# levi106/kvedge

Hardware: AMD Instinct MI355X
Metric: images/sec ResNet-50 edge module at 1/2/4/8 MI355X; VM boot-to-ready sec (higher is better)
Workload: dtype bf16; 1 GPU; model=resnet50, global_batch=1280, per_gpu_batch=1280, image_size=224, parallelism=dp1, backend=none, hip_graph=True, streams=2, microbatch=0, mb_blocks=3

## Files before the change

csrc/kernels/conv_seam.hip:

```cpp
#include "common.h"
#include "kvedge_kernels.h"

namespace kvedge {
namespace {

constexpr int kSmOOB = 0x7ffffff0;
constexpr int kSmLdsMax = 160 * 1024;

template <int I>
struct SmIC {
  static constexpr int value = I;
};
template <int N, int I = 0, class F>
__device__ __forceinline__ void sm_static_for(F&& f) {
  if constexpr (I < N) {
    f(SmIC<I>{});
    sm_static_for<N, I + 1>(f);
  }
}

template <int N>
__device__ __forceinline__ void sm_wait_vm() {
  static_assert(N >= 0 && N <= 63, "vmcnt field");
  asm volatile("s_waitcnt vmcnt(%0)" ::"n"(N) : "memory");
}

template <int SY, int SZ, int D, int RD, int KB, int NA>
struct SmSched {
  static constexpr int SPT = SY + SZ;
  static constexpr int kB = KB, kR = 2, kS = 2, kA = NA;
  static constexpr int kFar = 12;
  static constexpr int kTiles = kFar + 2;
  static constexpr int wait(int kind, int idx) {
    long endB[kTiles * SPT + D + 2] = {};
    long endR[kTiles + RD + 2] = {};
    long pos = kA;
    for (int t = 0; t < RD - 1; ++t) endR[t] = (pos += kR);
    for (int s = 0; s < D - 1; ++s) endB[s] = (pos += kB);
    for (int t = 0; t < kTiles; ++t) {
      for (int j = 0; j < SPT; ++j) {
        const int s = t * SPT + j;
        if (j == SY) {
          if (kind == 1 && idx == t) return (int)(pos - endR[t]);
          pos += kS;
        }
        if (kind == 0 && idx == s) return (int)(pos - endB[s]);
        if (kind == 2 && idx == s) return D >= 3 ? (int)(pos - endB[s + 1]) : -1;
        endB[s + D - 1] = (pos += kB);
        if (j == 0) endR[t + RD - 1] = (pos += kR);
      }
    }
    return -1;
  }
  static constexpr int wB(int t, int j) { return wait(0, t * SPT + j); }
  static constexpr int wE(int t) { return wait(1, t); }
  static constexpr int wXB(int t, int j) { return wait(2, t * SPT + j); }
  static constexpr int steady_from() {
    int t0 = 0;
    for (int t = 0; t < kFar; ++t) {
      bool same = wE(t) == wE(kFar);
      for (int j = 0; j < SPT; ++j)
        same = same && wB(t, j) == wB(kFar, j) && wXB(t, j) == wXB(kFar, j);
      if (!same) t0 = t + 1;
    }
    return t0;
  }
  static constexpr int kSteady = steady_from();
  static constexpr int safe_B(int j) {
    int m = wB(kFar, j);
    for (int t = 0; t <= kSteady; ++t) m = wB(t, j) < m ? wB(t, j) : m;
    return m;
  }
  static constexpr int safe_XB(int j) {
    int m = wXB(kFar, j);
    for (int t = 0; t <= kSteady; ++t) m = wXB(t, j) < m ? wXB(t, j) : m;
    return m;
  }
  static constexpr int safe_E() {
    int m = wE(kFar);
    for (int t = 0; t <= kSteady; ++t) m = wE(t) < m ? wE(t) : m;
    return m;
  }
  static constexpr bool ok(bool xp = false) {
    for (int t = 0; t <= kFar; ++t) {
      if (wE(t) < 0 || wE(t) > 63) return false;
      for (int j = 0; j < SPT; ++j) {
        if (wB(t, j) < 0 || wB(t, j) > 63) return false;
        if (xp && (wXB(t, j) < 0 || wXB(t, j) > 63)) return false;
      }
    }
    return kSteady < kFar;
  }
};

__device__ __forceinline__ int sm_sw(int r) { return (r >> 1) & 7; }

__device__ __forceinline__ void sm_lds_barrier() {
  asm volatile("s_waitcnt lgkmcnt(0)" ::: "memory");
  __builtin_amdgcn_s_barrier();
  asm volatile("" ::: "memory");
}

template <int NC3, int NZC, int D, int RD, int NW = 8, int KS2 = 1, bool AREG = false,
          bool XP = false>
__global__ __launch_bounds__(64 * NW, NW == 4 ? 2 : 1) void conv_seam_kernel(const KvConvParams p, int ntiles) {
  static_assert(NW == 4 || NW == 8, "waves");
  static_assert(NC3 % KS2 == 0 && NZC % KS2 == 0, "whole chunks per ring stage");
  constexpr int SY = NC3 / KS2, SZ = NZC / KS2, BPW = 8 / NW;
  using S = SmSched<SY, SZ, D, RD, KS2 * BPW, AREG ? 0 : 2 * NC3>;
  static_assert(S::ok(XP), "counted-wait schedule out of range or not periodic");
  constexpr int SPT = S::SPT, BM = 16 * NW, NT = 64 * NW;
  static_assert(!XP || (AREG && D >= 3 && SPT % 2 == 0),
                "XP: A in VGPRs, stage s + 1 issued before step s, register sets by step parity");
  constexpr int A_BYTES = AREG ? 0 : NC3 * BM * 128, B_CHUNK = 64 * 128, B_STAGE = KS2 * B_CHUNK;
  constexpr int R_SLOT = BM * 64 * 2;
  constexpr int B_OFF = A_BYTES, R_OFF = B_OFF + D * B_STAGE, BIAS_OFF = R_OFF + RD * R_SLOT;
  constexpr int BIAS_ROUND = NW * 1024;
  extern __shared__ __attribute__((aligned(16))) char sm_smem[];
  char* const lds = sm_smem;

  const int tid = threadIdx.x, lane = tid & 63;
  const int wv = __builtin_amdgcn_readfirstlane(tid >> 6);
  const int wm = wv >> 1, wn = wv & 1;
  const int nbm = (p.M + BM - 1) / BM;
  const int m0 = xcd_remap(blockIdx.x, nbm) * BM;
  const int Cout = p.Cout, N1 = p.n_t;
  const int b1_off = BIAS_OFF + ((Cout * 4 + BIAS_ROUND - 1) / BIAS_ROUND) * BIAS_ROUND;

  const kv_i32x4 rx = kv_rsrc4(p.x, p.M * p.ldx * 2);
  const kv_i32x4 rw3 = kv_rsrc4(p.w, Cout * p.Kpad * 2);
  const kv_i32x4 rw1 = kv_rsrc4(p.w_t, N1 * Cout * 2);
  const kv_i32x4 rr = kv_rsrc4(p.res, p.M * p.ldr * 2);
  const kv_i32x4 rb3 = kv_rsrc4(p.bias, Cout * 4);
  const kv_i32x4 rb1 = kv_rsrc4(p.bias_t, N1 * 4);
  const __amdgpu_buffer_rsrc_t ry =
      __builtin_amdgcn_make_buffer_rsrc(p.y, (short)0, p.M * p.ldy * 2, 0x00020000);
  const __amdgpu_buffer_rsrc_t rz =
      __builtin_amdgcn_make_buffer_rsrc(p.z, (short)0, p.M * p.ldz * 2, 0x00020000);

  const int lrow = lane >> 3, pch = lane & 7;
  int arow_off[2], r_src[2], lc8[2];
#pragma unroll
  for (int i = 0; i < 2; ++i) {
    const int row = (wv * 2 + i) * 8 + lrow;
    const int lc = pch ^ sm_sw(row);
    lc8[i] = lc * 8;
    const int m = m0 + row;
    arow_off[i] = m < p.M ? (m * p.ldx + p.x_coff + lc * 8) * 2 : kSmOOB;
    r_src[i] = m < p.M ? (m * p.ldr + p.r_coff + lc * 8) * 2 : kSmOOB;
  }
  int w3_src[BPW], w1_src[BPW], brow[BPW];
#pragma unroll
  for (int i = 0; i < BPW; ++i) {
    brow[i] = (wv * BPW + i) * 8 + lrow;
    const int bch = (pch ^ sm_sw(brow[i])) * 8;
    w3_src[i] = (brow[i] * p.Kpad + bch) * 2;
    w1_src[i] = (brow[i] * Cout + bch) * 2;
  }

  auto issue_B = [&](int tt, auto JJ) __attribute__((always_inline)) {
    constexpr int jj = decltype(JJ)::value;
    const int s = tt * SPT + jj;
    char* dst = lds + B_OFF + (s % D) * B_STAGE;
#pragma unroll
    for (int c = 0; c < KS2; ++c)
#pragma unroll
      for (int i = 0; i < BPW; ++i) {
        char* d = dst + c * B_CHUNK + (wv * BPW + i) * 1024;
        if constexpr (jj < SY) {
          const int n = tt * 64 + brow[i];
          const int v = (tt < ntiles && n < Cout) ? w3_src[i] + (tt * 64 * p.Kpad + (jj * KS2 + c) * 64) * 2 : kSmOOB;
          kv_lds_dma16(rw3, d, v);
        } else {
          const int zc = (jj - SY) * KS2 + c;
          const int zr = zc * 64 + brow[i];
          const int v = (tt < ntiles && zr < N1) ? w1_src[i] + (zc * 64 * Cout + tt * 64) * 2 : kSmOOB;
          kv_lds_dma16(rw1, d, v);
        }
      }
  };
  auto issue_R = [&](int tt) __attribute__((always_inline)) {
    char* dst = lds + R_OFF + (tt % RD) * R_SLOT;
#pragma unroll
    for (int i = 0; i < 2; ++i) {
      const int n = tt * 64 + lc8[i];
      const int v = (tt < ntiles && n < Cout && r_src[i] != kSmOOB) ? r_src[i] + tt * 128 : kSmOOB;
      kv_lds_dma16_nt(rr, dst + (wv * 2 + i) * 1024, v);
    }
  };

  for (int i = 0; i < (Cout * 4 + BIAS_ROUND - 1) / BIAS_ROUND; ++i) {
    const int off = (i * NW + wv) * 1024;
    kv_lds_dma16(rb3, lds + BIAS_OFF + off, off + lane * 16);
  }
  for (int i = 0; i < (N1 * 4 + BIAS_ROUND - 1) / BIAS_ROUND; ++i) {
    const int off = (i * NW + wv) * 1024;
    kv_lds_dma16(rb1, lds + b1_off + off, off + lane * 16);
  }
  typedef unsigned int sm_u32x4 __attribute__((ext_vector_type(4)));
  sm_u32x4 araw[AREG ? NC3 : 1][2][2];
  const int fr = lane & 15, fh = lane >> 4;
  if constexpr (AREG) {
#pragma unroll
    for (int kc = 0; kc < NC3; ++kc)
#pragma unroll
      for (int ks = 0; ks < 2; ++ks)
#pragma unroll
        for (int tm = 0; tm < 2; ++tm) {
          const int m = m0 + wm * 32 + tm * 16 + fr;
          const int k = kc * 64 + ks * 32 + fh * 8;
          const int off = (m < p.M && k < p.Cin) ? (m * p.ldx + p.x_coff + k) * 2 : kSmOOB;
          asm volatile("buffer_load_dwordx4 %0, %1, %2, 0 offen"
                       : "=v"(araw[kc][ks][tm]) : "v"(off), "s"(rx) : "memory");
        }
  }
  if constexpr (!AREG) {
#pragma unroll
    for (int kc = 0; kc < NC3; ++kc)
#pragma unroll
      for (int i = 0; i < 2; ++i) {
        char* dst = lds + kc * (BM * 128) + (wv * 2 + i) * 1024;
        const int v = (arow_off[i] != kSmOOB && kc * 64 + lc8[i] < p.Cin) ? arow_off[i] + kc * 128 : kSmOOB;
        kv_lds_dma16_nt(rx, dst, v);
      }
  }
#pragma unroll
  for (int t = 0; t < RD - 1; ++t) issue_R(t);
  sm_static_for<D - 1>([&](auto JJ) __attribute__((always_inline)) {
    constexpr int s = decltype(JJ)::value;
    issue_B(s / SPT, SmIC<s % SPT>{});
  });
  bf16x8 areg[AREG ? NC3 : 1][2][2];
  if constexpr (AREG) {
    sm_wait_vm<(RD - 1) * S::kR + (D - 1) * S::kB>();
#pragma unroll
    for (int kc = 0; kc < NC3; ++kc)
#pragma unroll
      for (int ks = 0; ks < 2; ++ks)
#pragma unroll
        for (int tm = 0; tm < 2; ++tm) {
          asm volatile("" : "+v"(araw[kc][ks][tm]));
          areg[kc][ks][tm] = __builtin_bit_cast(bf16x8, araw[kc][ks][tm]);
        }
  }

  floatx4 acc[2][2];
  floatx4 accz[NZC][2][2];
#pragma unroll
  for (int zc = 0; zc < NZC; ++zc)
#pragma unroll
    for (int a = 0; a < 2; ++a)
#pragma unroll
      for (int b = 0; b < 2; ++b) accz[zc][a][b] = floatx4{0.f, 0.f, 0.f, 0.f};

  auto mma64 = [&](const char* As, const char* Bs, floatx4 (&c)[2][2]) __attribute__((always_inline)) {
#pragma unroll
    for (int ks = 0; ks < 2; ++ks) {
      const int q = ks * 4 + fh;
      bf16x8 af[2], bfg[2];
#pragma unroll
      for (int tm = 0; tm < 2; ++tm) {
        const int row = wm * 32 + tm * 16 + fr;
        af[tm] = *reinterpret_cast<const bf16x8*>(As + row * 128 + ((q ^ sm_sw(row)) << 4));
      }
#pragma unroll
      for (int tn = 0; tn < 2; ++tn) {
        const int row = wn * 32 + tn * 16 + fr;
        bfg[tn] = *reinterpret_cast<const bf16x8*>(Bs + row * 128 + ((q ^ sm_sw(row)) << 4));
      }
#pragma unroll
      for (int tn = 0; tn < 2; ++tn)
#pragma unroll
        for (int tm = 0; tm < 2; ++tm)
          c[tn][tm] = __builtin_amdgcn_mfma_f32_16x16x32_bf16(bfg[tn], af[tm], c[tn][tm], 0, 0, 0);
    }
  };

  auto mma64r = [&](int kc_unused, const bf16x8 (&a)[2][2], const char* Bs, floatx4 (&c)[2][2])
      __attribute__((always_inline)) {
#pragma unroll
    for (int ks = 0; ks < 2; ++ks) {
      const int q = ks * 4 + fh;
      bf16x8 bfg[2];
#pragma unroll
      for (int tn = 0; tn < 2; ++tn) {
        const int row = wn * 32 + tn * 16 + fr;
        bfg[tn] = *reinterpret_cast<const bf16x8*>(Bs + row * 128 + ((q ^ sm_sw(row)) << 4));
      }
#pragma unroll
      for (int tn = 0; tn < 2; ++tn)
#pragma unroll
        for (int tm = 0; tm < 2; ++tm)
          c[tn][tm] = __builtin_amdgcn_mfma_f32_16x16x32_bf16(bfg[tn], a[ks][tm], c[tn][tm], 0, 0, 0);
    }
  };

  bf16x8 bset[XP ? 2 : 1][XP ? KS2 : 1][2][2];
  auto read_B = [&](bf16x8 (&dst)[XP ? KS2 : 1][2][2], const char* Bs) __attribute__((always_inline)) {
#pragma unroll
    for (int c = 0; c < (XP ? KS2 : 1); ++c)
#pragma unroll
      for (int ks = 0; ks < 2; ++ks)
#pragma unroll
        for (int tn = 0; tn < 2; ++tn) {
          const int row = wn * 32 + tn * 16 + fr, q = ks * 4 + fh;
          dst[c][ks][tn] =
              *reinterpret_cast<const bf16x8*>(Bs + c * B_CHUNK + row * 128 + ((q ^ sm_sw(row)) << 4));
        }
  };
  auto mma_xr = [&](const bf16x8 (&b)[2][2], const bf16x8 (&a)[2][2], floatx4 (&c)[2][2])
      __attribute__((always_inline)) {
#pragma unroll
    for (int ks = 0; ks < 2; ++ks)
#pragma unroll
      for (int tn = 0; tn < 2; ++tn)
#pragma unroll
        for (int tm = 0; tm < 2; ++tm)
          c[tn][tm] = __builtin_amdgcn_mfma_f32_16x16x32_bf16(b[ks][tn], a[ks][tm], c[tn][tm], 0, 0, 0);
  };
  auto mma_xl = [&](const bf16x8 (&b)[2][2], const char* As, floatx4 (&c)[2][2])
      __attribute__((always_inline)) {
#pragma unroll
    for (int ks = 0; ks < 2; ++ks) {
      const int q = ks * 4 + fh;
      bf16x8 af[2];
#pragma unroll
      for (int tm = 0; tm < 2; ++tm) {
        const int row = wm * 32 + tm * 16 + fr;
        af[tm] = *reinterpret_cast<const bf16x8*>(As + row * 128 + ((q ^ sm_sw(row)) << 4));
      }
#pragma unroll
      for (int tn = 0; tn < 2; ++tn)
#pragma unroll
        for (int tm = 0; tm < 2; ++tm)
          c[tn][tm] = __builtin_amdgcn_mfma_f32_16x16x32_bf16(b[ks][tn], af[tm], c[tn][tm], 0, 0, 0);
    }
  };

  dispatch_act(p.act, true, [&](auto A1, auto A2) __attribute__((always_inline)) {
    constexpr int act1 = decltype(A1)::value, act2 = decltype(A2)::value;
    for (int t = 0; t < ntiles; ++t) {
      const bool warm = t < S::kSteady;
      char* Rs = lds + R_OFF + (t % RD) * R_SLOT;
      sm_static_for<SPT>([&](auto JC) __attribute__((always_inline)) {
        constexpr int j = decltype(JC)::value;
        const int s = t * SPT + j;
        if constexpr (j == SY) {
          if (warm) sm_wait_vm<S::safe_E()>();
          else sm_wait_vm<S::wE(S::kFar)>();
          sm_lds_barrier();
          const float* bias_t = reinterpret_cast<const float*>(lds + BIAS_OFF) + t * 64;
#pragma unroll
          for (int tn = 0; tn < 2; ++tn) {
            const int c0 = wn * 32 + tn * 16 + fh * 4;
            const float4 bv = *reinterpret_cast<const float4*>(bias_t + c0);
#pragma unroll
            for (int tm = 0; tm < 2; ++tm) {
              const int row = wm * 32 + tm * 16 + fr;
              bf16x4* ptr = reinterpret_cast<bf16x4*>(Rs + row * 128 + (((c0 >> 3) ^ sm_sw(row)) << 4) +
                                                      (c0 & 7) * 2);
              const bf16x4 rv = *ptr;
              bf16x4 o;
              o[0] = f2bf(act_c<act2>(act_c<act1>(acc[tn][tm][0] + bv.x) + (float)rv[0]));
              o[1] = f2bf(act_c<act2>(act_c<act1>(acc[tn][tm][1] + bv.y) + (float)rv[1]));
              o[2] = f2bf(act_c<act2>(act_c<act1>(acc[tn][tm][2] + bv.z) + (float)rv[2]));
              o[3] = f2bf(act_c<act2>(act_c<act1>(acc[tn][tm][3] + bv.w) + (float)rv[3]));
              *ptr = o;
            }
          }
          sm_lds_barrier();
#pragma unroll
          for (int i = 0; i < 2; ++i) {
            const int idx = tid + NT * i;
            const int row = idx >> 3, c = idx & 7;
            const bf16x8 v = *reinterpret_cast<const bf16x8*>(Rs + row * 128 + ((c ^ sm_sw(row)) << 4));
            const int m = m0 + row, n = t * 64 + c * 8;
            const int off = (m < p.M && n < Cout) ? (m * p.ldy + p.y_coff + n) * 2 : kSmOOB;
            __builtin_amdgcn_raw_buffer_store_b128(__builtin_bit_cast(kv_i32x4, v), ry, off, 0, 2);
          }
        }
        if constexpr (j == 0) {
#pragma unroll
          for (int a = 0; a < 2; ++a)
#pragma unroll
            for (int b = 0; b < 2; ++b) acc[a][b] = floatx4{0.f, 0.f, 0.f, 0.f};
        }
        if constexpr (XP) {
          if (warm) sm_wait_vm<S::safe_XB(j)>();
          else sm_wait_vm<S::wXB(S::kFar, j)>();
        } else {
          if (warm) sm_wait_vm<S::safe_B(j)>();
          else sm_wait_vm<S::wB(S::kFar, j)>();
        }
        sm_lds_barrier();
        constexpr int jn = (j + D - 1) % SPT, tadv = (j + D - 1) / SPT;
        issue_B(t + tadv, SmIC<jn>{});
        if constexpr (j == 0) issue_R(t + RD - 1);
        const char* Bs = lds + B_OFF + (s % D) * B_STAGE;
        if constexpr (XP) {
          constexpr int cur = j & 1, nxt = cur ^ 1;
          if constexpr (j == 0) {
            if (t == 0) read_B(bset[cur], Bs);
          }
          read_B(bset[nxt], lds + B_OFF + ((s + 1) % D) * B_STAGE);
#pragma unroll
          for (int c = 0; c < KS2; ++c) {
            if constexpr (j < SY) mma_xr(bset[cur][c], areg[j * KS2 + c], acc);
            else mma_xl(bset[cur][c], Rs, accz[(j - SY) * KS2 + c]);
          }
        } else {
#pragma unroll
          for (int c = 0; c < KS2; ++c) {
            if constexpr (j < SY && AREG) mma64r(0, areg[j * KS2 + c], Bs + c * B_CHUNK, acc);
            else if constexpr (j < SY) mma64(lds + (j * KS2 + c) * (BM * 128), Bs + c * B_CHUNK, acc);
            else mma64(Rs, Bs + c * B_CHUNK, accz[(j - SY) * KS2 + c]);
          }
        }
      });
    }
  });

  asm volatile("s_waitcnt vmcnt(0)" ::: "memory");
  __syncthreads();
  const float* b1 = reinterpret_cast<const float*>(lds + b1_off);
  const bool relu_z = p.act_t == 1;
  sm_static_for<NZC>([&](auto ZC) __attribute__((always_inline)) {
    constexpr int zc = decltype(ZC)::value;
    char* Zs = lds + R_OFF + (zc % RD) * R_SLOT;
    if constexpr (zc > 0 && zc % RD == 0) __syncthreads();
#pragma unroll
    for (int tn = 0; tn < 2; ++tn) {
      const int c0 = wn * 32 + tn * 16 + fh * 4;
      const float4 bv = *reinterpret_cast<const float4*>(b1 + zc * 64 + c0);
#pragma unroll
      for (int tm = 0; tm < 2; ++tm) {
        const int row = wm * 32 + tm * 16 + fr;
        float v0 = accz[zc][tn][tm][0] + bv.x, v1 = accz[zc][tn][tm][1] + bv.y;
        float v2 = accz[zc][tn][tm][2] + bv.z, v3 = accz[zc][tn][tm][3] + bv.w;
        if (relu_z) {
          v0 = fmaxf(v0, 0.f); v1 = fmaxf(v1, 0.f); v2 = fmaxf(v2, 0.f); v3 = fmaxf(v3, 0.f);
        }
        bf16x4 o;
        o[0] = f2bf(v0); o[1] = f2bf(v1); o[2] = f2bf(v2); o[3] = f2bf(v3);
        *reinterpret_cast<bf16x4*>(Zs + row * 128 + (((c0 >> 3) ^ sm_sw(row)) << 4) + (c0 & 7) * 2) = o;
      }
    }
    if constexpr (zc % RD == RD - 1 || zc == NZC - 1) {
      __syncthreads();
      constexpr int z0 = zc - zc % RD;
#pragma unroll
      for (int g = z0; g <= zc; ++g) {
        const char* Zg = lds + R_OFF + (g % RD) * R_SLOT;
#pragma unroll
        for (int i = 0; i < 2; ++i) {
          const int idx = tid + NT * i;
          const int row = idx >> 3, c = idx & 7;
          const bf16x8 v = *reinterpret_cast<const bf16x8*>(Zg + row * 128 + ((c ^ sm_sw(row)) << 4));
          const int m = m0 + row, n = g * 64 + c * 8;
          const int off = (m < p.M && n < N1) ? (m * p.ldz + p.z_coff + n) * 2 : kSmOOB;
          __builtin_amdgcn_raw_buffer_store_b128(__builtin_bit_cast(kv_i32x4, v), rz, off, 0, 0);
        }
      }
    }
  });
}

typedef void (*SmFn)(const KvConvParams, int);

struct SmTile {
  int nc3, nzc, d, rd, nw, ks2, areg;
  SmFn fn;
};

template <int NC3, int NZC, int D, int RD, int NW = 8, int KS2 = 1, bool AREG = false,
          bool XP = false>
constexpr SmTile sm_tile() {
  return SmTile{NC3, NZC, D, RD, NW, KS2, AREG ? 1 : 0,
                &conv_seam_kernel<NC3, NZC, D, RD, NW, KS2, AREG, XP>};
}

static const SmTile kSmTiles[] = {
    sm_tile<2, 2, 4, 3, 4>(),
    sm_tile<2, 2, 6, 3>(),
    sm_tile<2, 2, 4, 3, 8, 2>(),
    sm_tile<2, 2, 6, 3, 4, 1, true>(),
    sm_tile<2, 2, 6, 3, 8, 2, true>(),
    sm_tile<2, 4, 6, 3, 8, 2, true>(),
    sm_tile<2, 4, 6, 3>(),
    sm_tile<4, 4, 4, 4, 8, 2, true, true>(),
    sm_tile<4, 4, 4, 4, 8, 2, true>(),
    sm_tile<4, 4, 3, 2, 8, 2>(),
    sm_tile<4, 4, 5, 2>(),
    sm_tile<4, 4, 3, 2, 4>(),
    sm_tile<4, 4, 6, 2, 8, 2, true>(),
    sm_tile<4, 4, 8, 3, 8, 1, true>(),
    sm_tile<4, 4, 3, 5, 8, 2, true>(),
    sm_tile<4, 8, 4, 3>(),
};

int sm_lds_bytes(const SmTile& e, int cout, int n1) {
  const int bm = 16 * e.nw, round = e.nw * 1024;
  return (e.areg ? 0 : e.nc3 * bm * 128) + e.d * e.ks2 * 64 * 128 + e.rd * bm * 128 +
         ((cout * 4 + round - 1) / round) * round + ((n1 * 4 + round - 1) / round) * round;
}

}

int seam_num_tiles() { return (int)(sizeof(kSmTiles) / sizeof(kSmTiles[0])); }

int seam_pick_tile(const KvConvParams* p) {
  for (int i = 0; i < seam_num_tiles(); ++i) {
    const SmTile& e = kSmTiles[i];
    if (p->Kpad == e.nc3 * 64 && p->n_t == e.nzc * 64 && sm_lds_bytes(e, p->Cout, p->n_t) <= kSmLdsMax)
      return i;
  }
  return -1;
}

int seam_launch(const KvConvParams* p, int tile, hipStream_t stream) {
  if (tile < 0 || tile >= seam_num_tiles()) return -6;
  const SmTile& e = kSmTiles[tile];
  if (p->mode != 1 || !p->res || p->x2 || !p->w_t || !p->z || p->in_u8 || p->pair_1x1) return -8;
  if (p->Kpad != e.nc3 * 64 || p->Cin > p->Kpad || p->n_t != e.nzc * 64 || p->Cout % 64) return -8;
  if (p->ldx % 8 || p->x_coff % 8 || p->ldy % 8 || p->y_coff % 8 || p->ldr % 8 || p->r_coff % 8 ||
      p->ldz % 8 || p->z_coff % 8 || p->x_coff + p->Cin > p->ldx || p->y_coff + p->Cout > p->ldy ||
      p->r_coff + p->Cout > p->ldr || p->z_coff + p->n_t > p->ldz)
    return -8;
  if ((long long)p->M * p->ldy * 2 >= kSmOOB || (long long)p->M * p->ldr * 2 >= kSmOOB ||
      (long long)p->M * p->ldx * 2 >= kSmOOB || (long long)p->M * p->ldz * 2 >= kSmOOB ||
      (long long)p->Cout * p->Kpad * 2 >= kSmOOB || (long long)p->n_t * p->Cout * 2 >= kSmOOB)
    return -9;
  const int lds = sm_lds_bytes(e, p->Cout, p->n_t);
  if (lds > kSmLdsMax) return -11;
  const int nbm = (p->M + 16 * e.nw - 1) / (16 * e.nw), ntiles = p->Cout / 64;
  if (nbm <= 0 || ntiles <= 0) return 0;
  if (hipFuncSetAttribute(reinterpret_cast<const void*>(e.fn),
                          hipFuncAttributeMaxDynamicSharedMemorySize, lds) != hipSuccess)
    return -7;
  hipLaunchKernelGGL(e.fn, dim3((unsigned)nbm), dim3(64 * e.nw), (unsigned)lds, stream, *p, ntiles);
  return hipGetLastError() == hipSuccess ? 0 : -7;
}

}
```

kvedge_amd/models/resnet.py:

```python
from __future__ import annotations

import os

from typing import List, Optional

import torch
import torch.nn as nn
import torch.nn.functional as F

from .. import ops
from .layers import (DeployedConv, DeployedDualConv, calibrate_bn, count_flops, fold_bn,
                     frames_to_nchw)

ACT_NONE, ACT_RELU = ops.ACT_NONE, ops.ACT_RELU
TAIL1_MIN_ROWS = int(os.environ.get("KVEDGE_TAIL1_MIN_ROWS", "32768"))


class Bottleneck(nn.Module):
    expansion = 4

    def __init__(self, cin: int, width: int, stride: int):
        super().__init__()
        cout = width * self.expansion
        self.conv1 = nn.Conv2d(cin, width, 1, bias=False)
        self.bn1 = nn.BatchNorm2d(width)
        self.conv2 = nn.Conv2d(width, width, 3, stride, 1, bias=False)
        self.bn2 = nn.BatchNorm2d(width)
        self.conv3 = nn.Conv2d(width, cout, 1, bias=False)
        self.bn3 = nn.BatchNorm2d(cout)
        self.downsample = None
        if stride != 1 or cin != cout:
            self.downsample = nn.Sequential(nn.Conv2d(cin, cout, 1, stride, bias=False),
                                            nn.BatchNorm2d(cout))

    def forward(self, x):
        idt = x if self.downsample is None else self.downsample(x)
        y = F.relu(self.bn1(self.conv1(x)))
        y = F.relu(self.bn2(self.conv2(y)))
        y = self.bn3(self.conv3(y))
        return F.relu(y + idt)


class ResNet50Ref(nn.Module):
    layers_cfg = ((64, 3, 1), (128, 4, 2), (256, 6, 2), (512, 3, 2))

    def __init__(self, num_classes: int = 1000):
        super().__init__()
        self.conv1 = nn.Conv2d(3, 64, 7, 2, 3, bias=False)
        self.bn1 = nn.BatchNorm2d(64)
        blocks: List[nn.Module] = []
        cin = 64
        for width, n, stride in self.layers_cfg:
            for i in range(n):
                blocks.append(Bottleneck(cin, width, stride if i == 0 else 1))
                cin = width * 4
        self.blocks = nn.Sequential(*blocks)
        self.fc = nn.Linear(2048, num_classes)
        self.num_classes = num_classes

    def forward(self, x):
        x = F.relu(self.bn1(self.conv1(x)))
        x = F.max_pool2d(x, 3, 2, 1)
        x = self.blocks(x)
        x = torch.flatten(F.adaptive_avg_pool2d(x, 1), 1)
        return self.fc(x)


def init_resnet50(seed: int = 0, num_classes: int = 1000, calibrate: bool = True,
                  calib_batch: int = 4, calib_hw: int = 224) -> ResNet50Ref:
    g = torch.Generator().manual_seed(seed)
    m = ResNet50Ref(num_classes)
    for mod in m.modules():
        if isinstance(mod, nn.Conv2d):
            fan_out = mod.out_channels * mod.kernel_size[0] * mod.kernel_size[1]
            with torch.no_grad():
                mod.weight.normal_(0.0, (2.0 / fan_out) ** 0.5, generator=g)
        elif isinstance(mod, nn.BatchNorm2d):
            nn.init.ones_(mod.weight)
            nn.init.zeros_(mod.bias)
        elif isinstance(mod, nn.Linear):
            bound = 1.0 / mod.in_features ** 0.5
            with torch.no_grad():
                mod.weight.uniform_(-bound, bound, generator=g)
                mod.bias.uniform_(-bound, bound, generator=g)
    if calibrate:
        frames = torch.randint(0, 256, (calib_batch, calib_hw, calib_hw, 3), generator=g,
                               dtype=torch.uint8)
        calibrate_bn(m, [frames_to_nchw(frames)])
    m.eval()
    return m


class DeployedBottleneck:

    def __init__(self, b: Bottleneck, device, fuse_down: bool = True):
        self.c1 = DeployedConv.from_modules(b.conv1, b.bn1, ACT_RELU, device)
        self.c2 = DeployedConv.from_modules(b.conv2, b.bn2, ACT_RELU, device)
        self.c3 = DeployedConv.from_modules(b.conv3, b.bn3, ACT_RELU, device)
        self.down = None
        self.dual = None
        if b.downsample is not None:
            self.down = DeployedConv.from_modules(b.downsample[0], b.downsample[1], ACT_NONE,
                                                  device)
            if fuse_down:
                self.dual = DeployedDualConv.from_modules(b.conv3, b.bn3, b.downsample[0],
                                                          b.downsample[1], ACT_RELU, device)

    def __call__(self, x, out=None, t1=None):
        y = self.c1(x) if t1 is None else t1
        y = self.c2(y)
        if self.dual is not None:
            return self.dual(y, x, out=out)
        idt = x if self.down is None else self.down(x)
        return self.c3(y, res=idt, out=out)

    def can_tail(self, nxt: "DeployedBottleneck") -> bool:
        c1 = nxt.c1.spec
        cout = self.c3.spec.cout
        if not (c1.kh == 1 and c1.stride == 1 and c1.pad == 0 and c1.cin == cout and
                c1.act == ACT_RELU and self.c3.spec.act == ACT_RELU):
            return False
        if cout != 256:
            k3 = self.c3.spec.cin
            return (ops.SEAM_ENABLED and self.down is None and self.dual is None and
                    (k3, cout, c1.cout) in ops.SEAM_SHAPES)
        k = self.c3.spec.cin + (self.dual.w.shape[1] - self.dual.k1 if self.dual is not None else 0)
        return (c1.cout in (64, 128) and (self.dual is not None or self.down is None) and
                (self.dual is None or c1.cout == 64) and k <= 128)

    def tail_fits(self, x: torch.Tensor, batch: int = 0) -> bool:
        N, Ho, Wo, _ = self.out_shape(x.shape)
        N = batch or N
        if self.c3.spec.cout == 256:
            return N * Ho * Wo >= TAIL1_MIN_ROWS
        return (N * Ho * Wo + 127) // 128 >= ops.SEAM_MIN_WGS

    def call_tail(self, x, nxt: "DeployedBottleneck", t1=None, out=None, z=None):
        y = self.c1(x) if t1 is None else t1
        y = self.c2(y)
        c1 = nxt.c1
        if self.dual is not None:
            d = self.dual
            return ops.conv_tail(y, d.w, d.b, d.act, c1.w, c1.b, x2=x, stride2=d.stride2,
                                 out=out, z=z)
        return ops.conv_tail(y, self.c3.w, self.c3.b, self.c3.spec.act, c1.w, c1.b, res=x,
                             out=out, z=z)

    def out_shape(self, x_shape):
        N, H, W, _ = x_shape
        Ho, Wo = self.c2.spec.out_hw(H, W)
        return (N, Ho, Wo, self.c3.spec.cout)

    def convs(self):
        return [c for c in (self.c1, self.c2, self.c3, self.down, self.dual) if c is not None]


class KvResNet50:

    image_size = 224

    def __init__(self, ref: ResNet50Ref, device="cuda"):
        self.device = torch.device(device)
        self.num_classes = ref.num_classes
        self.stem = DeployedConv.stem_s2d(ref.conv1, ref.bn1, ACT_RELU, self.device)
        wf, _ = fold_bn(ref.conv1, ref.bn1)
        self.stem12_w = ops.pack_stem12(wf).to(self.device)
        self._flops = {}
        self._ref = ref
        self.blocks = [DeployedBottleneck(b, self.device) for b in ref.blocks]
        fcw = ref.fc.weight.detach().float()[:, :, None, None]
        fc_conv = nn.Conv2d(2048, ref.num_classes, 1, bias=True)
        with torch.no_grad():
            fc_conv.weight.copy_(fcw)
            fc_conv.bias.copy_(ref.fc.bias.detach())
        self.fc = DeployedConv.from_modules(fc_conv, None, ACT_NONE, self.device)

    @staticmethod
    def build(seed: int = 0, device="cuda", calibrate: bool = True) -> "KvResNet50":
        return KvResNet50(init_resnet50(seed, calibrate=calibrate), device)

    def convs(self) -> List[DeployedConv]:
        out = [self.stem]
        for b in self.blocks:
            out += b.convs()
        return out + [self.fc]

    def flops_per_image(self, hw: int = 224) -> int:
        if hw not in self._flops:
            self._flops[hw] = count_flops(self._ref, (1, 3, hw, hw))
        return self._flops[hw]

    def frame_plan(self, src_hw, image_size: int = 0) -> "ops.ResizePlan":
        return ops.center_crop_plan(src_hw, image_size or self.image_size)

    def preprocess(self, frames_u8: torch.Tensor) -> torch.Tensor:
        return ops.preprocess(frames_u8, s2d=True)

    microbatch: int = 0
    microbatch_blocks: int = 3
    fuse_stem_pool: bool = True
    fuse_preprocess: bool = True
    fuse_tail: bool = True
    stem12: bool = True

    def stem_and_pool(self, x: torch.Tensor, frames_in: bool = False) -> torch.Tensor:
        if frames_in:
            if self.stem12:
                return ops.stem12_pool_frames(x, self.stem12_w, self.stem.b)
            return ops.stem_pool_frames(x, self.stem.spec, self.stem.w, self.stem.b)
        if self.fuse_stem_pool:
            return ops.stem_pool(x, self.stem.spec, self.stem.w, self.stem.b)
        return ops.maxpool2d(self.stem(x), 3, 2, 1)

    def features(self, x: torch.Tensor, frames_in: bool = False) -> torch.Tensor:
        B = x.shape[0]
        mb = self.microbatch
        nb = self.microbatch_blocks
        t1 = None
        if mb and B > mb and B % mb == 0 and 0 < nb < len(self.blocks):
            full = full_t1 = None
            for i in range(0, B, mb):
                y = self.stem_and_pool(x[i:i + mb], frames_in)
                z = None
                for j in range(nb):
                    b, nxt = self.blocks[j], self.blocks[j + 1]
                    last = j == nb - 1
                    if last and full is None:
                        shp = b.out_shape(y.shape)
                        full = ops.empty((B,) + shp[1:], dtype=y.dtype, device=y.device)
                    fuse = (self.fuse_tail and y.is_cuda and b.can_tail(nxt) and
                            b.tail_fits(y, batch=B))
                    if last and full_t1 is None and fuse:
                        full_t1 = ops.empty(full.shape[:3] + (nxt.c1.spec.cout,),
                                            dtype=y.dtype, device=y.device)
                    o = full[i:i + mb] if last else None
                    if fuse:
                        y, z = b.call_tail(y, nxt, t1=z, out=o,
                                           z=full_t1[i:i + mb] if last else None)
                    else:
                        y, z = b(y, t1=z, out=o), None
            x, t1 = full, full_t1
            rest = self.blocks[nb:]
        else:
            x = self.stem_and_pool(x, frames_in)
            rest = self.blocks
        for i, b in enumerate(rest):
            nxt = rest[i + 1] if i + 1 < len(rest) else None
            if (self.fuse_tail and x.is_cuda and nxt is not None and b.can_tail(nxt) and
                    b.tail_fits(x)):
                x, t1 = b.call_tail(x, nxt, t1=t1)
            else:
                x, t1 = b(x, t1=t1), None
        return x

    def logits(self, x: torch.Tensor, frames_in: bool = False) -> torch.Tensor:
        f = self.features(x, frames_in)
        B = f.shape[0]
        if f.is_cuda and B <= ops.POOLED_FC_MAX_BATCH and self.fuse_head:
            return ops.pooled_fc(f, self.fc.w, self.fc.b)
        pooled = ops.global_avgpool(f).view(B, 1, 1, 2048)
        return self.fc(pooled).view(B, self.num_classes)

    fuse_head: bool = os.environ.get("KVEDGE_FUSE_HEAD", "0") == "1"

    def raw_outputs(self, frames_u8: torch.Tensor) -> torch.Tensor:
        if self.fuse_preprocess and self.fuse_stem_pool and frames_u8.is_cuda:
            return self.logits(frames_u8, frames_in=True)
        return self.logits(self.preprocess(frames_u8))

    def __call__(self, frames_u8: torch.Tensor, out: Optional[dict] = None):
        lg = self.raw_outputs(frames_u8)
        probs, top1 = ops.softmax_rows(lg)
        return probs, top1
```

kvedge_amd/ops/__init__.py:

```python
from __future__ import annotations

import os
from dataclasses import dataclass
from typing import Optional, Sequence, Tuple

import torch

from . import reference as _ref

_LIB_PATH = os.path.join(os.path.dirname(os.path.dirname(os.path.abspath(__file__))),
                         "_C_checks.so" if os.environ.get("KVEDGE_CHECKS", "0") not in ("", "0")
                         else os.path.basename(os.environ.get("KVEDGE_LIB", "") or "_C.so"))
_loaded = False
_load_error: Optional[str] = None

ACT_NONE, ACT_RELU, ACT_SILU = 0, 1, 2
RES_AFTER_ACT = 4
MODE_GENERAL, MODE_GEMM, MODE_STEM = 0, 1, 2
BK = 64


def load(build_if_missing: bool = False) -> bool:
    global _loaded, _load_error
    if _loaded:
# ... 103 lines not shown
    @staticmethod
    def auto(cin, cout, k, stride=1, pad=None, act=ACT_NONE) -> "ConvSpec":
        if pad is None:
            pad = k // 2
        if cin < 8:
            mode = MODE_STEM
        elif k == 1 and stride == 1 and pad == 0:
            mode = MODE_GEMM
        else:
            mode = MODE_GENERAL
        return ConvSpec(cin, cout, k, k, stride, pad, act, mode)


def pack_conv_weight(w: torch.Tensor, spec: ConvSpec) -> torch.Tensor:
    assert w.shape == (spec.cout, spec.cin, spec.kh, spec.kw), (w.shape, spec)
    w = w.detach().float()
    if spec.mode == MODE_STEM:
        wp = torch.zeros(spec.cout, spec.kh, spec.kwp, 4, dtype=torch.float32, device=w.device)
        wp[:, :, :spec.kw, :spec.cin] = w.permute(0, 2, 3, 1)
        flat = wp.reshape(spec.cout, -1)
    else:
        flat = w.permute(0, 2, 3, 1).reshape(spec.cout, -1)
    out = torch.zeros(spec.cout, spec.Kpad, dtype=torch.float32, device=w.device)
    out[:, :flat.shape[1]] = flat
    return out.to(torch.bfloat16).contiguous()


def unpack_conv_weight(wp: torch.Tensor, spec: ConvSpec) -> torch.Tensor:
    wf = wp.float()[:, :spec.K]
    if spec.mode == MODE_STEM:
        w4 = wf.reshape(spec.cout, spec.kh, spec.kwp, 4)[:, :, :spec.kw, :spec.cin]
        return w4.permute(0, 3, 1, 2).contiguous()
    return wf.reshape(spec.cout, spec.kh, spec.kw, spec.cin).permute(0, 3, 1, 2).contiguous()


_WS: dict = {}
SPLITK_MAX_ELEMS = 32 << 20
SPLITK_MAX_SPLIT = 32
N_SPLITK_TILES = 19
N_DE_TILES = 3
N_SKINNY_TILES = 9
SPLITK0 = 1 << 30


def is_splitk(tile: int) -> bool:
    return SPLITK0 <= tile < SPLITK0 + N_SPLITK_TILES


def splitk_workspace(device: torch.device, elems: int) -> Optional[torch.Tensor]:
    if elems > SPLITK_MAX_ELEMS // 2:
        return None
    key = (device.index, torch.cuda.current_stream(device).cuda_stream)
    ws = _WS.get(key)
    if ws is None:
        ws = torch.empty(SPLITK_MAX_ELEMS, dtype=torch.float32, device=device)
        _WS[key] = ws
    return ws


def conv2d(x: torch.Tensor, spec: ConvSpec, w: torch.Tensor, bias: Optional[torch.Tensor],
           res: Optional[torch.Tensor] = None, out: Optional[torch.Tensor] = None,
           x_coff: int = 0, y_coff: int = 0, r_coff: int = 0, tile: int = -1) -> torch.Tensor:
    N, H, W, ldx = x.shape
    Ho, Wo = spec.out_hw(H, W)
    if out is None:
        out = empty(N, Ho, Wo, spec.cout, dtype=torch.bfloat16, device=x.device)
    assert out.shape[:3] == (N, Ho, Wo), (out.shape, (N, Ho, Wo))
    ldy = out.shape[3]
    ldr = res.shape[-1] if res is not None else 0
    if (res is not None and res.data_ptr() == out.data_ptr() and ldr == ldy
            and r_coff < y_coff + spec.cout and y_coff < r_coff + spec.cout):
        raise ValueError(f"kvedge: residual slice [{r_coff}, {r_coff + spec.cout}) and output "
                         f"slice [{y_coff}, {y_coff + spec.cout}) of one buffer overlap")
    if x.is_cuda:
        ws = splitk_workspace(x.device, N * Ho * Wo * spec.cout) if is_splitk(tile) else None
        _native().conv(x, w, bias, res, out, N, H, W, spec.cin_eff, ldx, x_coff, Ho, Wo,
                       spec.cout, spec.kh, spec.kw, spec.stride, spec.pad, spec.K, ldy, y_coff,
                       ldr, r_coff, spec.act, spec.mode, tile, ws)
    else:
        _ref.conv2d(x, spec, w, bias, res, out, x_coff, y_coff, r_coff)
    return out


def conv_pair(x: torch.Tensor, spec: ConvSpec, w: torch.Tensor, bias: torch.Tensor,
              w2: torch.Tensor, b2: torch.Tensor, out: torch.Tensor, x_coff: int = 0,
              z_coff: int = 0, tile: int = 0) -> torch.Tensor:
    assert spec.kh == 3 and spec.stride == 1 and spec.pad == 1 and spec.mode == MODE_GENERAL
    C2 = w2.shape[0]
    assert w2.shape[1] == spec.cout and out.shape[:3] == x.shape[:3]
    if x.is_cuda:
        _native().conv_pair(x, w, bias, w2, b2, out, spec.cin, x_coff, z_coff, spec.act, tile)
        return out
    t = torch.empty(*x.shape[:3], spec.cout, dtype=torch.bfloat16)
    _ref.conv2d(x, spec, w, bias, None, t, x_coff, 0, 0)
    z = t.float() @ w2.float().t() + b2.float()
    out[..., z_coff:z_coff + C2] = z.to(out.dtype)
    return out


def conv_dual(x1: torch.Tensor, x2: torch.Tensor, w: torch.Tensor, bias: Optional[torch.Tensor],
              act: int, stride2: int, out: Optional[torch.Tensor] = None,
              tile: int = -1) -> torch.Tensor:
    N, Ho, Wo, K1 = x1.shape
    cout = w.shape[0]
    if out is None:
        out = empty(N, Ho, Wo, cout, dtype=torch.bfloat16, device=x1.device)
    if x1.is_cuda:
        ws = splitk_workspace(x1.device, N * Ho * Wo * cout) if is_splitk(tile) else None
        _native().conv_dual(x1, x2, w, bias, out, stride2, act, tile, ws)
    else:
        _ref.conv_dual(x1, x2, w, bias, act, stride2, out)
    return out


def conv_dual2(x: torch.Tensor, K1: int, x2: torch.Tensor, w: torch.Tensor,
               bias: Optional[torch.Tensor], act: int, out: torch.Tensor, x_coff: int = 0,
               x2_coff: int = 0, y_coff: int = 0, stride2: int = 1, up2: bool = False,
               tile: int = -1) -> torch.Tensor:
    if x.is_cuda:
        N, Ho, Wo, _ = x.shape
        ws = splitk_workspace(x.device, N * Ho * Wo * w.shape[0]) if is_splitk(tile) else None
        _native().conv_dual2(x, x_coff, K1, x2, x2_coff, w, bias, out, y_coff, stride2,
                             1 if up2 else 0, act, tile, ws)
    else:
        _ref.conv_dual2(x, x_coff, K1, x2, x2_coff, w, bias, act, stride2, up2, out, y_coff)
    return out


def conv_tail(x: torch.Tensor, w: torch.Tensor, bias: Optional[torch.Tensor], act: int,
              w1: torch.Tensor, b1: Optional[torch.Tensor], res: Optional[torch.Tensor] = None,
              x2: Optional[torch.Tensor] = None, stride2: int = 1,
              out: Optional[torch.Tensor] = None, z: Optional[torch.Tensor] = None,
              tile: int = -1):
    N, H, W, _ = x.shape
    cout, nt = w.shape[0], w1.shape[0]
    if out is None:
        out = empty(N, H, W, cout, dtype=torch.bfloat16, device=x.device)
    if z is None:
        z = empty(N, H, W, nt, dtype=torch.bfloat16, device=x.device)
    if x.is_cuda:
        _native().conv_tail(x, x2, w, bias, res, out, w1, b1, z, stride2, act, tile)
        return out, z
    if x2 is not None:
        _ref.conv_dual(x, x2, w, bias, act, stride2, out)
    else:
        spec = ConvSpec.auto(x.shape[3], cout, 1, 1, 0, act)
        _ref.conv2d(x, spec, w, bias, res, out, 0, 0, 0)
    spec1 = ConvSpec.auto(cout, nt, 1, 1, 0, ACT_RELU)
    _ref.conv2d(out, spec1, w1, b1, None, z, 0, 0, 0)
    return out, z


SEAM_SHAPES = {(128, 512, 128), (128, 512, 256), (256, 1024, 256)}
SEAM_ENABLED = os.environ.get("KVEDGE_SEAM", "1") != "0"
SEAM_MIN_WGS = int(os.environ.get("KVEDGE_SEAM_MIN_WGS", "256"))


C2F_ENABLED = os.environ.get("KVEDGE_C2F", "1") != "0"


def c2f16_strip(H: int, W: int) -> int:
    for S in (40, 32, 20, 16, 8, 4):
        if H % S == 0 and W in (80, 160):
            return S
    return 0


def c2f16(x: torch.Tensor, w1: torch.Tensor, b1: torch.Tensor, wm1: torch.Tensor,
          bm1: torch.Tensor, wm2: torch.Tensor, bm2: torch.Tensor, w2: torch.Tensor,
          b2: torch.Tensor, out: Optional[torch.Tensor] = None, x_coff: int = 0,
          y_coff: int = 0, S: int = 0) -> torch.Tensor:
    N, H, W, _ = x.shape
    if out is None:
        out = empty(N, H, W, 32, dtype=torch.bfloat16, device=x.device)
    if x.is_cuda:
        _native().c2f16_fused(x, x_coff, w1, b1, wm1, bm1, wm2, bm2, w2, b2, out, y_coff,
                              S or c2f16_strip(H, W))
        return out
    s1 = ConvSpec.auto(32, 32, 1, 1, 0, ACT_SILU)
    sm1 = ConvSpec.auto(16, 16, 3, 1, 1, ACT_SILU)
    sm2 = ConvSpec.auto(16, 16, 3, 1, 1, ACT_SILU | RES_AFTER_ACT)
    s2 = ConvSpec.auto(48, 32, 1, 1, 0, ACT_SILU)
    cat = torch.empty(N, H, W, 48, dtype=torch.bfloat16)
    u = torch.empty(N, H, W, 16, dtype=torch.bfloat16)
    _ref.conv2d(x, s1, w1, b1, None, cat, x_coff, 0, 0)
    _ref.conv2d(cat, sm1, wm1, bm1, None, u, 16, 0, 0)
    _ref.conv2d(u, sm2, wm2, bm2, cat, cat, 0, 32, 16)
    _ref.conv2d(cat, s2, w2, b2, None, out, 0, y_coff, 0)
    return out


def stem_pool(x: torch.Tensor, spec: "ConvSpec", w: torch.Tensor, bias: torch.Tensor,
              out: Optional[torch.Tensor] = None, y_coff: int = 0) -> torch.Tensor:
    assert spec.cin == 16 and spec.cout == 64 and spec.kh == 4 and spec.stride == 1
    assert spec.pad == 2 and spec.pad_end == 1 and spec.act == ACT_RELU and spec.Kpad == 256
    N, H, W, _ = x.shape
    Hp, Wp = (H - 1) // 2 + 1, (W - 1) // 2 + 1
    if out is None:
        out = empty(N, Hp, Wp, 64, dtype=torch.bfloat16, device=x.device)
    if x.is_cuda:
        _native().stem_pool(x, w, bias, out, y_coff)
    else:
        y = conv2d(x, spec, w, bias)
        maxpool2d(y, 3, 2, 1, out=out, y_coff=y_coff)
    return out


def stem_pool_frames(frames: torch.Tensor, spec: "ConvSpec", w: torch.Tensor,
                     bias: torch.Tensor, out: Optional[torch.Tensor] = None, y_coff: int = 0,
                     mean=None, std=None) -> torch.Tensor:
    assert frames.dtype == torch.uint8 and frames.dim() == 4 and frames.shape[3] == 3
    mean = IMAGENET_MEAN if mean is None else mean
    std = IMAGENET_STD if std is None else std
    if not frames.is_cuda:
        return stem_pool(preprocess(frames, mean=mean, std=std, s2d=True), spec, w, bias,
                         out=out, y_coff=y_coff)
    assert spec.cin == 16 and spec.cout == 64 and spec.kh == 4 and spec.stride == 1
    assert spec.pad == 2 and spec.pad_end == 1 and spec.act == ACT_RELU and spec.Kpad == 256
    N, H0, W0, _ = frames.shape
    H, W = H0 // 2, W0 // 2
    if out is None:
        out = empty(N, (H - 1) // 2 + 1, (W - 1) // 2 + 1, 64, dtype=torch.bfloat16,
                    device=frames.device)
    _native().stem_pool_frames(frames, w, bias, out, list(mean), list(std), y_coff)
    return out


def pack_stem12(wf: torch.Tensor) -> torch.Tensor:
    cout, cin, k, _ = wf.shape
    assert cin == 3 and k == 7
    w = torch.zeros(cout, 4, 4, 2, 2, 3)
    for r in range(4):
        for dy in range(2):
            ky = 2 * r - 1 + dy
            if not 0 <= ky < 7:
                continue
            for s_ in range(4):
                for dx in range(2):
                    kx = 2 * s_ - 1 + dx
                    if 0 <= kx < 7:
                        w[:, r, s_, dy, dx, :] = wf[:, :, ky, kx].float()
    return w.reshape(cout, 192).to(torch.bfloat16).contiguous()


def stem12_reference(frames: torch.Tensor, w12: torch.Tensor, bias: torch.Tensor,
                     mean=None, std=None) -> torch.Tensor:
    mean = IMAGENET_MEAN if mean is None else mean
    std = IMAGENET_STD if std is None else std
    N, H0, W0, _ = frames.shape
    Hs, Ws = H0 // 2, W0 // 2
    m = torch.tensor(mean, dtype=torch.float32)
    inv = 1.0 / torch.tensor(std, dtype=torch.float32)
    x = (frames.float() * (inv / 255.0) + (-m * inv)).to(torch.bfloat16).float()
    x = x.view(N, Hs, 2, Ws, 2, 3).permute(0, 1, 3, 2, 4, 5).reshape(N, Hs, Ws, 12)
    xp = torch.nn.functional.pad(x, (0, 0, 2, 1, 2, 1))
    cols = xp.unfold(1, 4, 1).unfold(2, 4, 1)
    cols = cols.permute(0, 1, 2, 4, 5, 3).reshape(N, Hs, Ws, 192)
    y = cols @ w12.float().t() + bias.float()
    y = y.to(torch.bfloat16).float().relu()
    y = torch.nn.functional.max_pool2d(y.permute(0, 3, 1, 2), 3, 2, 1).permute(0, 2, 3, 1)
    return y.to(torch.bfloat16).contiguous()


def stem12_pool_frames(frames: torch.Tensor, w12: torch.Tensor, bias: torch.Tensor,
                       out: Optional[torch.Tensor] = None, y_coff: int = 0,
                       mean=None, std=None) -> torch.Tensor:
    assert frames.dtype == torch.uint8 and frames.dim() == 4 and frames.shape[3] == 3
    mean = IMAGENET_MEAN if mean is None else mean
    std = IMAGENET_STD if std is None else std
    N, H0, W0, _ = frames.shape
    Hs, Ws = H0 // 2, W0 // 2
    if out is None:
        out = empty(N, (Hs - 1) // 2 + 1, (Ws - 1) // 2 + 1, 64, dtype=torch.bfloat16,
                    device=frames.device)
    if not frames.is_cuda:
        out[..., y_coff:y_coff + 64] = stem12_reference(frames, w12, bias, mean, std)
        return out
    _native().stem12_pool_frames(frames, w12, bias, out, list(mean), list(std), y_coff)
    return out


def yolo_stem2_fits(frames_shape) -> bool:
    _, H, W, _ = frames_shape
    return H % 4 == 0 and W % 32 == 0 and 0 < W <= 640


def yolo_stem2(frames: torch.Tensor, spec0: "ConvSpec", w0: torch.Tensor, b0: torch.Tensor,
               spec1: "ConvSpec", w1: torch.Tensor, b1: torch.Tensor,
               out: Optional[torch.Tensor] = None) -> torch.Tensor:
    assert spec0.kh == 2 and spec0.cin == 16 and spec0.cout == 16, spec0
    assert (spec1.kh, spec1.stride, spec1.cin, spec1.cout) == (3, 2, 16, 32), spec1
    assert spec0.act == ACT_SILU and spec1.act == ACT_SILU
    N, H, W, _ = frames.shape
    if out is None:
        out = empty(N, H // 4, W // 4, 32, dtype=torch.bfloat16, device=frames.device)
    if not frames.is_cuda:
        x = stem_from_frames(frames, spec0, w0, b0)
        return conv2d(x, spec1, w1, b1, out=out)
    _native().yolo_stem2(frames, w0, b0, w1, b1, out)
    return out


def stem_from_frames(frames: torch.Tensor, spec: "ConvSpec", w: torch.Tensor,
                     bias: Optional[torch.Tensor], out: Optional[torch.Tensor] = None,
                     tile: int = -1) -> torch.Tensor:
    assert spec.kh == 2 and spec.stride == 1 and spec.cin == 16, spec
# ... 597 lines not shown
```

Before: 88130 images/sec.

## Add dual-source seam kernel fusing downsample block tail with next block's 1x1

Extends the seam conv kernel with a dual-source mode: the A operand is assembled in LDS from two inputs, the block's own activations plus a strided gather of the block input (the projection shortcut folded into one GEMM). The result then feeds the next block's first 1x1 conv in the same kernel. The residual ring loads and their counted waits are skipped in this mode, and a new tile config is added for the (128,256,512,128) shape. The model now routes downsample blocks to this path when the shape matches and the grid is large enough, saving an intermediate write and read plus a launch, at the cost of more kernel variants and a stricter occupancy threshold.

```diff
diff --git a/csrc/kernels/conv_seam.hip b/csrc/kernels/conv_seam.hip
--- a/csrc/kernels/conv_seam.hip
+++ b/csrc/kernels/conv_seam.hip
@@ -25,13 +25,14 @@
   asm volatile("s_waitcnt vmcnt(%0)" ::"n"(N) : "memory");
 }
 
-template <int SY, int SZ, int D, int RD, int KB, int NA>
+template <int SY, int SZ, int D, int RD, int KB, int NA, int KR = 2>
 struct SmSched {
   static constexpr int SPT = SY + SZ;
-  static constexpr int kB = KB, kR = 2, kS = 2, kA = NA;
+  static constexpr int kB = KB, kR = KR, kS = 2, kA = NA;
   static constexpr int kFar = 12;
   static constexpr int kTiles = kFar + 2;
   static constexpr int wait(int kind, int idx) {
+    if (kind == 1 && KR == 0) return 0;
     long endB[kTiles * SPT + D + 2] = {};
     long endR[kTiles + RD + 2] = {};
     long pos = kA;
@@ -102,12 +103,14 @@
 }
 
 template <int NC3, int NZC, int D, int RD, int NW = 8, int KS2 = 1, bool AREG = false,
-          bool XP = false>
+          bool XP = false, int NC1 = 0>
 __global__ __launch_bounds__(64 * NW, NW == 4 ? 2 : 1) void conv_seam_kernel(const KvConvParams p, int ntiles) {
   static_assert(NW == 4 || NW == 8, "waves");
   static_assert(NC3 % KS2 == 0 && NZC % KS2 == 0, "whole chunks per ring stage");
+  constexpr bool DUAL = NC1 > 0;
+  static_assert(!DUAL || (NC1 < NC3 && !AREG && !XP), "dual form: two sources, A in LDS");
   constexpr int SY = NC3 / KS2, SZ = NZC / KS2, BPW = 8 / NW;
-  using S = SmSched<SY, SZ, D, RD, KS2 * BPW, AREG ? 0 : 2 * NC3>;
+  using S = SmSched<SY, SZ, D, RD, KS2 * BPW, AREG ? 0 : 2 * NC3, DUAL ? 0 : 2>;
   static_assert(S::ok(XP), "counted-wait schedule out of range or not periodic");
   constexpr int SPT = S::SPT, BM = 16 * NW, NT = 64 * NW;
   static_assert(!XP || (AREG && D >= 3 && SPT % 2 == 0),
@@ -130,7 +133,8 @@
   const kv_i32x4 rx = kv_rsrc4(p.x, p.M * p.ldx * 2);
   const kv_i32x4 rw3 = kv_rsrc4(p.w, Cout * p.Kpad * 2);
   const kv_i32x4 rw1 = kv_rsrc4(p.w_t, N1 * Cout * 2);
-  const kv_i32x4 rr = kv_rsrc4(p.res, p.M * p.ldr * 2);
+  const kv_i32x4 rr = kv_rsrc4(DUAL ? p.x2 : p.res,
+                               DUAL ? p.N * p.H2 * p.W2 * p.ldx2 * 2 : p.M * p.ldr * 2);
   const kv_i32x4 rb3 = kv_rsrc4(p.bias, Cout * 4);
   const kv_i32x4 rb1 = kv_rsrc4(p.bias_t, N1 * 4);
   const __amdgpu_buffer_rsrc_t ry =
@@ -147,7 +151,13 @@
     lc8[i] = lc * 8;
     const int m = m0 + row;
     arow_off[i] = m < p.M ? (m * p.ldx + p.x_coff + lc * 8) * 2 : kSmOOB;
-    r_src[i] = m < p.M ? (m * p.ldr + p.r_coff + lc * 8) * 2 : kSmOOB;
+    if constexpr (DUAL) {
+      const int hw = p.Ho * p.Wo, n = m / hw, rem = m - n * hw, ho = rem / p.Wo, wo = rem - ho * p.Wo;
+      const int px = (n * p.H2 + ho * p.stride2) * p.W2 + wo * p.stride2;
+      r_src[i] = m < p.M ? (px * p.ldx2 + p.x2_coff + lc * 8) * 2 : kSmOOB;
+    } else {
+      r_src[i] = m < p.M ? (m * p.ldr + p.r_coff + lc * 8) * 2 : kSmOOB;
+    }
   }
   int w3_src[BPW], w1_src[BPW], brow[BPW];
 #pragma unroll
@@ -220,12 +230,18 @@
 #pragma unroll
       for (int i = 0; i < 2; ++i) {
         char* dst = lds + kc * (BM * 128) + (wv * 2 + i) * 1024;
-        const int v = (arow_off[i] != kSmOOB && kc * 64 + lc8[i] < p.Cin) ? arow_off[i] + kc * 128 : kSmOOB;
-        kv_lds_dma16_nt(rx, dst, v);
-      }
-  }
-#pragma unroll
-  for (int t = 0; t < RD - 1; ++t) issue_R(t);
+        if (DUAL && kc >= NC1) {
+          kv_lds_dma16(rr, dst, r_src[i] != kSmOOB ? r_src[i] + (kc - NC1) * 128 : kSmOOB);
+        } else {
+          const int v = (arow_off[i] != kSmOOB && kc * 64 + lc8[i] < p.Cin) ? arow_off[i] + kc * 128 : kSmOOB;
+          kv_lds_dma16_nt(rx, dst, v);
+        }
+      }
+  }
+  if constexpr (!DUAL) {
+#pragma unroll
+    for (int t = 0; t < RD - 1; ++t) issue_R(t);
+  }
   sm_static_for<D - 1>([&](auto JJ) __attribute__((always_inline)) {
     constexpr int s = decltype(JJ)::value;
     issue_B(s / SPT, SmIC<s % SPT>{});
@@ -337,7 +353,7 @@
     }
   };
 
-  dispatch_act(p.act, true, [&](auto A1, auto A2) __attribute__((always_inline)) {
+  dispatch_act(p.act, !DUAL, [&](auto A1, auto A2) __attribute__((always_inline)) {
     constexpr int act1 = decltype(A1)::value, act2 = decltype(A2)::value;
     for (int t = 0; t < ntiles; ++t) {
       const bool warm = t < S::kSteady;
@@ -346,8 +362,10 @@
         constexpr int j = decltype(JC)::value;
         const int s = t * SPT + j;
         if constexpr (j == SY) {
-          if (warm) sm_wait_vm<S::safe_E()>();
-          else sm_wait_vm<S::wE(S::kFar)>();
+          if constexpr (!DUAL) {
+            if (warm) sm_wait_vm<S::safe_E()>();
+            else sm_wait_vm<S::wE(S::kFar)>();
+          }
           sm_lds_barrier();
           const float* bias_t = reinterpret_cast<const float*>(lds + BIAS_OFF) + t * 64;
 #pragma unroll
@@ -359,7 +377,8 @@
               const int row = wm * 32 + tm * 16 + fr;
               bf16x4* ptr = reinterpret_cast<bf16x4*>(Rs + row * 128 + (((c0 >> 3) ^ sm_sw(row)) << 4) +
                                                       (c0 & 7) * 2);
-              const bf16x4 rv = *ptr;
+              bf16x4 rv = {};
+              if constexpr (!DUAL) rv = *ptr;
               bf16x4 o;
               o[0] = f2bf(act_c<act2>(act_c<act1>(acc[tn][tm][0] + bv.x) + (float)rv[0]));
               o[1] = f2bf(act_c<act2>(act_c<act1>(acc[tn][tm][1] + bv.y) + (float)rv[1]));
@@ -395,7 +414,7 @@
         sm_lds_barrier();
         constexpr int jn = (j + D - 1) % SPT, tadv = (j + D - 1) / SPT;
         issue_B(t + tadv, SmIC<jn>{});
-        if constexpr (j == 0) issue_R(t + RD - 1);
+        if constexpr (j == 0 && !DUAL) issue_R(t + RD - 1);
         const char* Bs = lds + B_OFF + (s % D) * B_STAGE;
         if constexpr (XP) {
           constexpr int cur = j & 1, nxt = cur ^ 1;
@@ -468,15 +487,15 @@
 typedef void (*SmFn)(const KvConvParams, int);
 
 struct SmTile {
-  int nc3, nzc, d, rd, nw, ks2, areg;
+  int nc3, nzc, d, rd, nw, ks2, areg, nc1;
   SmFn fn;
 };
 
 template <int NC3, int NZC, int D, int RD, int NW = 8, int KS2 = 1, bool AREG = false,
-          bool XP = false>
+          bool XP = false, int NC1 = 0>
 constexpr SmTile sm_tile() {
-  return SmTile{NC3, NZC, D, RD, NW, KS2, AREG ? 1 : 0,
-                &conv_seam_kernel<NC3, NZC, D, RD, NW, KS2, AREG, XP>};
+  return SmTile{NC3, NZC, D, RD, NW, KS2, AREG ? 1 : 0, NC1,
+                &conv_seam_kernel<NC3, NZC, D, RD, NW, KS2, AREG, XP, NC1>};
 }
 
 static const SmTile kSmTiles[] = {
@@ -496,6 +515,7 @@
     sm_tile<4, 4, 8, 3, 8, 1, true>(),
     sm_tile<4, 4, 3, 5, 8, 2, true>(),
     sm_tile<4, 8, 4, 3>(),
+    sm_tile<6, 2, 4, 1, 8, 1, false, false, 2>(),
 };
 
 int sm_lds_bytes(const SmTile& e, int cout, int n1) {
@@ -511,6 +531,7 @@
 int seam_pick_tile(const KvConvParams* p) {
   for (int i = 0; i < seam_num_tiles(); ++i) {
     const SmTile& e = kSmTiles[i];
+    if ((p->x2 != nullptr) != (e.nc1 > 0) || (p->x2 && p->K1 != e.nc1 * 64)) continue;
     if (p->Kpad == e.nc3 * 64 && p->n_t == e.nzc * 64 && sm_lds_bytes(e, p->Cout, p->n_t) <= kSmLdsMax)
       return i;
   }
@@ -520,11 +541,22 @@
 int seam_launch(const KvConvParams* p, int tile, hipStream_t stream) {
   if (tile < 0 || tile >= seam_num_tiles()) return -6;
   const SmTile& e = kSmTiles[tile];
-  if (p->mode != 1 || !p->res || p->x2 || !p->w_t || !p->z || p->in_u8 || p->pair_1x1) return -8;
+  if (!p->w_t || !p->z || p->in_u8 || p->pair_1x1) return -8;
+  if (e.nc1 > 0) {
+    if (p->mode != 4 || p->res || !p->x2 || p->up2 || p->stride2 < 1) return -8;
+    if (p->K1 != e.nc1 * 64 || p->Cin != p->K1 || p->K != p->Kpad) return -8;
+    if ((p->H2 + p->stride2 - 1) / p->stride2 != p->Ho || (p->W2 + p->stride2 - 1) / p->stride2 != p->Wo ||
+        p->M != p->N * p->Ho * p->Wo)
+      return -8;
+    if (p->ldx2 % 8 || p->x2_coff % 8 || p->x2_coff + (p->Kpad - p->K1) > p->ldx2) return -8;
+    if ((long long)p->N * p->H2 * p->W2 * p->ldx2 * 2 >= kSmOOB) return -9;
+  } else {
+    if (p->mode != 1 || !p->res || p->x2) return -8;
+  }
   if (p->Kpad != e.nc3 * 64 || p->Cin > p->Kpad || p->n_t != e.nzc * 64 || p->Cout % 64) return -8;
   if (p->ldx % 8 || p->x_coff % 8 || p->ldy % 8 || p->y_coff % 8 || p->ldr % 8 || p->r_coff % 8 ||
       p->ldz % 8 || p->z_coff % 8 || p->x_coff + p->Cin > p->ldx || p->y_coff + p->Cout > p->ldy ||
-      p->r_coff + p->Cout > p->ldr || p->z_coff + p->n_t > p->ldz)
+      (p->res && p->r_coff + p->Cout > p->ldr) || p->z_coff + p->n_t > p->ldz)
     return -8;
   if ((long long)p->M * p->ldy * 2 >= kSmOOB || (long long)p->M * p->ldr * 2 >= kSmOOB ||
       (long long)p->M * p->ldx * 2 >= kSmOOB || (long long)p->M * p->ldz * 2 >= kSmOOB ||
diff --git a/kvedge_amd/models/resnet.py b/kvedge_amd/models/resnet.py
--- a/kvedge_amd/models/resnet.py
+++ b/kvedge_amd/models/resnet.py
@@ -128,12 +128,29 @@
         return (c1.cout in (64, 128) and (self.dual is not None or self.down is None) and
                 (self.dual is None or c1.cout == 64) and k <= 128)
 
+    def can_seam_dual(self, nxt: "DeployedBottleneck") -> bool:
+        c1 = nxt.c1.spec
+        cout = self.c3.spec.cout
+        if self.dual is None or cout == 256 or not ops.SEAM_ENABLED:
+            return False
+        if not (c1.kh == 1 and c1.stride == 1 and c1.pad == 0 and c1.cin == cout and
+                c1.act == ACT_RELU and self.dual.act == ACT_RELU):
+            return False
+        k2 = self.dual.w.shape[1] - self.dual.k1
+        return (self.dual.k1, k2, cout, c1.cout) in ops.SEAM_DUAL_SHAPES
+
+    def can_fuse(self, nxt: "DeployedBottleneck") -> bool:
+        return self.can_tail(nxt) or self.can_seam_dual(nxt)
+
     def tail_fits(self, x: torch.Tensor, batch: int = 0) -> bool:
         N, Ho, Wo, _ = self.out_shape(x.shape)
         N = batch or N
         if self.c3.spec.cout == 256:
             return N * Ho * Wo >= TAIL1_MIN_ROWS
-        return (N * Ho * Wo + 127) // 128 >= ops.SEAM_MIN_WGS
+        wgs = (N * Ho * Wo + 127) // 128
+        if self.dual is not None:
+            return wgs >= 2 * ops.SEAM_MIN_WGS
+        return wgs >= ops.SEAM_MIN_WGS
 
     def call_tail(self, x, nxt: "DeployedBottleneck", t1=None, out=None, z=None):
         y = self.c1(x) if t1 is None else t1
@@ -228,7 +245,7 @@
                     if last and full is None:
                         shp = b.out_shape(y.shape)
                         full = ops.empty((B,) + shp[1:], dtype=y.dtype, device=y.device)
-                    fuse = (self.fuse_tail and y.is_cuda and b.can_tail(nxt) and
+                    fuse = (self.fuse_tail and y.is_cuda and b.can_fuse(nxt) and
                             b.tail_fits(y, batch=B))
                     if last and full_t1 is None and fuse:
                         full_t1 = ops.empty(full.shape[:3] + (nxt.c1.spec.cout,),
@@ -246,7 +263,7 @@
             rest = self.blocks
         for i, b in enumerate(rest):
             nxt = rest[i + 1] if i + 1 < len(rest) else None
-            if (self.fuse_tail and x.is_cuda and nxt is not None and b.can_tail(nxt) and
+            if (self.fuse_tail and x.is_cuda and nxt is not None and b.can_fuse(nxt) and
                     b.tail_fits(x)):
                 x, t1 = b.call_tail(x, nxt, t1=t1)
             else:
diff --git a/kvedge_amd/ops/__init__.py b/kvedge_amd/ops/__init__.py
--- a/kvedge_amd/ops/__init__.py
+++ b/kvedge_amd/ops/__init__.py
@@ -279,6 +279,7 @@
 
 
 SEAM_SHAPES = {(128, 512, 128), (128, 512, 256), (256, 1024, 256)}
+SEAM_DUAL_SHAPES = {(128, 256, 512, 128)}
 SEAM_ENABLED = os.environ.get("KVEDGE_SEAM", "1") != "0"
 SEAM_MIN_WGS = int(os.environ.get("KVEDGE_SEAM_MIN_WGS", "256"))
 
```

New measurement: 88820 images/sec, median of 6. No clear change (+0.8%).
